# lmb-freiburg/demon

Measured on AMD Instinct MI355X. Metric: image-pairs/s full 3-iter DeMoN forward @256x192, higher is better.
Workload: dtype f32

## Files before the change

### demon_amd/_lib.py

```python
import ctypes
import os

HERE = os.path.dirname(os.path.abspath(__file__))
LIB_PATH = os.environ.get("DEMON_HIP_LIB", os.path.join(HERE, "libdemon_hip.so"))

c_float_p = ctypes.POINTER(ctypes.c_float)
c_int_p = ctypes.POINTER(ctypes.c_int)
c_int64_p = ctypes.POINTER(ctypes.c_int64)
c_uint8_p = ctypes.POINTER(ctypes.c_uint8)


class DemonOutputs(ctypes.Structure):
    _fields_ = [(name, c_float_p) for name in (
        "predict_flow5", "predict_conf5", "predict_flow2", "predict_conf2", "predict_depth2",
        "predict_normal2", "predict_rotation", "predict_translation", "predict_scale")]


class LanesEntry(ctypes.Structure):
    _fields_ = [("lanes", ctypes.c_int), ("placeholder_streams", ctypes.c_int), ("pairs_per_s", ctypes.c_float)]


class LanesResult(ctypes.Structure):
    _fields_ = [("lanes", ctypes.c_int), ("placeholder_streams", ctypes.c_int), ("pairs_per_s", ctypes.c_float),
                ("verified_pairs_per_s", ctypes.c_float), ("attempts", ctypes.c_int), ("ntable", ctypes.c_int), ("table", LanesEntry * 64)]
# ... 62 lines not shown
    "demon_upload_images_u8_async": (_I, [_P, _I, c_uint8_p, c_uint8_p]),
    "demon_op_prepare_inputs_u8": (_I, [_P, c_float_p, c_float_p, c_uint8_p, c_uint8_p, _I, _I, _I, _I, _I]),
    "demon_cloud_configure": (_I, [_P, ctypes.POINTER(ctypes.c_double), _I]),
    "demon_run_cloud": (_I, [_P, _I]),
    "demon_download_cloud": (_I, [_P, _I, c_float_p, c_float_p, c_uint8_p, c_int_p]),
    "demon_download_cloud_async": (_I, [_P, _I, c_float_p, c_float_p, c_uint8_p, c_int_p]),
    "demon_download_outputs_async": (_I, [_P, _I, ctypes.POINTER(DemonOutputs), c_float_p]),
    "demon_host_register": (_I, [ctypes.c_void_p, ctypes.c_int64]),
    "demon_host_unregister": (_I, [ctypes.c_void_p]),
    "demon_time_full": (_I, [_P, _I, _I, _I, c_float_p]),
    "demon_profile_full": (_I, [_P, _I, _I, _I, ctypes.POINTER(LaunchRecord), _I, c_int_p]),
    "demon_op_depth_to_flow": (_I, [_P, c_float_p, c_float_p, c_float_p, c_float_p, c_float_p, _I, _I, _I, _I, _I, _I]),
    "demon_op_flow_to_depth": (_I, [_P, c_float_p, c_float_p, c_float_p, c_float_p, c_float_p, _I, _I, _I, _I, _I, _I]),
    "demon_op_warp2d": (_I, [_P, c_float_p, c_float_p, c_float_p, _I, _I, _I, _I, _I, _I, _F]),
    "demon_op_leaky_relu": (_I, [_P, c_float_p, c_float_p, ctypes.c_int64, _F]),
    "demon_op_replace_nonfinite": (_I, [_P, c_float_p, c_float_p, ctypes.c_int64, _F]),
    "demon_op_scale_invariant_gradient": (_I, [_P, c_float_p, c_float_p, _I, _I, _I, c_int_p, c_float_p, _I, _F]),
    "demon_op_median3x3_downsample": (_I, [_P, c_float_p, c_float_p, _I, _I, _I]),
    "demon_op_depth_to_normals": (_I, [_P, c_float_p, c_float_p, c_float_p, _I, _I, _I, _I]),
    "demon_op_pointwise_l2_loss": (_I, [_P, c_float_p, c_float_p, c_float_p, _I, _I, _I, _I, ctypes.c_float]),
    "demon_op_conv2d": (_I, [_P, c_float_p, c_float_p, c_float_p, c_float_p] + [_I] * 12),
    "demon_op_deconv4x4s2": (_I, [_P, c_float_p, c_float_p, c_float_p, c_float_p] + [_I] * 6),
    "demon_op_dense": (_I, [_P, c_float_p, c_float_p, c_float_p, c_float_p] + [_I] * 4),
    "demon_op_point_cloud": (_I, [_P, c_float_p, c_float_p, c_uint8_p, c_int_p, c_float_p, c_float_p, c_uint8_p, c_float_p, c_float_p, c_float_p, c_float_p] + [_I] * 5),
    "demon_bench_layer": (_I, [_P] + [_I] * 13 + [c_float_p, ctypes.POINTER(ctypes.c_double)]),
    "demon_bench_ingest": (_I, [_P, _I, _I, _I, c_float_p, c_float_p]),
    "demon_bench_cloud": (_I, [_P, _I, _I, _I, c_float_p]),
    "demon_last_kernel": (_I, [ctypes.c_char_p, _I]),
    "demon_debug_check_guards": (_I, [_P, c_int_p]),
}

_lib = None


def load():
    global _lib
    if _lib is not None:
        return _lib
    if not os.path.exists(LIB_PATH):
        raise RuntimeError(
            "libdemon_hip.so not found at %s -- build it with `python -m demon_amd.build` "
            "(there is no CPU fallback for the DeMoN hot path)" % LIB_PATH)
    lib = ctypes.CDLL(LIB_PATH)
    for name, (restype, argtypes) in SIGNATURES.items():
        fn = getattr(lib, name)
        fn.restype = restype
# ... 4 lines not shown
```

### demon_amd/build.py

```python
import os
import subprocess
import sys
from concurrent.futures import ThreadPoolExecutor

HERE = os.path.dirname(os.path.abspath(__file__))
CSRC = os.path.join(HERE, "csrc")
OUT = os.path.join(HERE, "libdemon_hip.so")
SOURCES = ["demon_api.hip", "conv_mfma.hip", "conv_bf16.hip", "conv_patch.hip", "conv_small.hip", "conv_pair.hip", "conv_stream.hip", "conv_frag.hip", "conv_wino.hip", "conv_wino3.hip", "conv_wino4.hip", "dense_stream.hip", "conv_thin.hip", "conv_row.hip", "ops.hip", "ingest.hip", "pointcloud.hip"]
FLAGS = ["--offload-arch=gfx950", "-O3", "-std=c++17", "-fPIC", "-Wall", "-Wno-unused-function", "-Wno-unused-value", "-Wno-unused-result"]


def csrc_sha():
    import glob
    import hashlib
    h = hashlib.sha1()
    files = [os.path.join(CSRC, n) for n in sorted(SOURCES) if n != "demon_api.hip"] + [os.path.join(CSRC, "internal.h"), os.path.join(CSRC, "wino1d_tables.h")]
    files += sorted(glob.glob(os.path.join(HERE, "tuned", "*.json")))
    for path in files:
        with open(path, "rb") as f:
            h.update(f.read())
    return h.hexdigest()[:16]


def _hipcc():
    for cand in (os.environ.get("HIPCC"), "/opt/rocm/bin/hipcc", "hipcc"):
        if cand and (os.path.isabs(cand) and os.path.exists(cand) or not os.path.isabs(cand)):
            return cand
    return "hipcc"


def _needs_build(target, deps):
# ... 47 lines not shown
```

### demon_amd/csrc/conv_pair.hip

```cpp
#include "internal.h"

namespace demon {

typedef float floatx16 __attribute__((ext_vector_type(16)));
typedef float floatx4 __attribute__((ext_vector_type(4)));

template <int K, int S, int MB1, int MB2, int C1>
struct PairGeom {
    static constexpr int TH = 4, TW = 32;
    static constexpr int TWm = (TW - 1) * S + K;
    static constexpr int TWp = (TWm + 3) / 4 * 4;
    static constexpr int PH = (TH - 1) * S + K;
    static constexpr int N1 = TH * TWp;
    static constexpr int NB1 = (N1 + 31) / 32;
    static constexpr int NBW = (NB1 + 3) / 4;
    static constexpr int CKS1 = C1;
    static constexpr bool ONE1 = C1 == 6;
    static constexpr int CKS2 = K == 3 ? 8 : 2;
    static constexpr int KD1 = K * CKS1, KD2 = K * CKS2;
    static constexpr int PPS = PH * TWp;
    static constexpr int PELEMS = CKS1 * PPS;
    static constexpr int EPP = (PPS + 255) / 256;
    static constexpr int A1CH = KD1 * MB1 * 8, A1PER = (A1CH + 255) / 256;
    static constexpr int A2CH = KD2 * MB2 * 8, A2PER = (A2CH + 255) / 256;
// ... 246 lines not shown
                float v = acc2[i][r] + a.b2[co];
                v = v >= 0.0f ? v : 0.1f * v;
                ob[(long)co * plane] = v;
            }
        }
}

template <int K, int S, int MB1, int MB2, int C1>
static bool launch_pair_t(const PairArgs &a_in, hipStream_t s)
{
    using G = PairGeom<K, S, MB1, MB2, C1>;
    static PerDeviceOnce once;
    if (G::lds_bytes > 64 * 1024 &&
        !once.ensure([] { return hipFuncSetAttribute(reinterpret_cast<const void *>(&conv_pair_kernel<K, S, MB1, MB2, C1>), hipFuncAttributeMaxDynamicSharedMemorySize, (int)G::lds_bytes) == hipSuccess; }))
        return false;
    PairArgs a = a_in;
    a.steps1 = (a.Cin + C1 - 1) / C1;
    a.steps2 = (a.CM + G::CKS2 - 1) / G::CKS2;
    dim3 grid((unsigned)(a.N * a.tiles_y * a.tiles_x));
    hipLaunchKernelGGL((conv_pair_kernel<K, S, MB1, MB2, C1>), grid, dim3(256), G::lds_bytes, s, a);
    return true;
}

bool conv_pair_applies(int k, int stride, int cin, int cm, int co)
{
    static const int all = getenv("DEMON_FUSED_PAIRS_ALL") ? atoi(getenv("DEMON_FUSED_PAIRS_ALL")) : 0;
    const bool shape = (k == 9 && stride == 2) || (k == 7 && stride == 2) || (k == 3 && stride == 1);
    if (!shape || cm > 64 || co > 64 || cm % 8) return false;
    return all || (k == 9 && cin <= 16);
}

void conv_pair_tiles(int Ho, int Wo, int &tiles_y, int &tiles_x)
{
    tiles_y = (Ho + 3) / 4;
    tiles_x = (Wo + 31) / 32;
}

int conv_pair_cks(int k) { return k == 3 ? 8 : 2; }

bool launch_conv_pair(const PairArgs &a, int k, int stride, hipStream_t s)
{
    const int mb1 = (a.CM + 31) / 32, mb2 = (a.CO + 31) / 32;
    static const int one_step = getenv("DEMON_PAIR_ONE_STEP") ? atoi(getenv("DEMON_PAIR_ONE_STEP")) : 1;
    if (k == 9 && stride == 2 && a.Cin == 6 && mb1 == 1 && one_step) {
        if (mb2 == 1) return launch_pair_t<9, 2, 1, 1, 6>(a, s);
        return launch_pair_t<9, 2, 1, 2, 6>(a, s);
    }
#define PAIR_CASE(KK, SS, CC)                                                  \
    if (k == KK && stride == SS) {                                             \
        if (mb1 == 1 && mb2 == 1) return launch_pair_t<KK, SS, 1, 1, CC>(a, s); \
        if (mb1 == 1 && mb2 == 2) return launch_pair_t<KK, SS, 1, 2, CC>(a, s); \
        if (mb1 == 2 && mb2 == 1) return launch_pair_t<KK, SS, 2, 1, CC>(a, s); \
// ... 11 lines not shown
```

### demon_amd/csrc/demon_api.hip

```cpp
#include <hip/hip_runtime.h>
#include <dlfcn.h>
#include <rccl/rccl.h>
#include <stdio.h>
#include <stdlib.h>
#include <string.h>

#include <algorithm>
#include <cmath>
#include <array>
#include <chrono>
#include <functional>
#include <mutex>
#include <map>
#include <memory>
#include <string>
#include <vector>

#include "../../include/demon_hip.h"
#include "internal.h"

using namespace demon;

namespace {

// ... 1234 lines not shown
    if (const char *pk = getenv("DEMON_TUNE_PICK")) {
        const Cand &cd = cands[(size_t)atoi(pk) % cands.size()];
        best_t = Layer::Tuned{cd.kind, cd.tile, cd.ksplit};
    }
    L->tuned[n] = best_t;
    return DEMON_OK;
}

bool run_pair(const Layer *Ly, const Layer *Lx, int n, hipStream_t s)
{
    PairArgs a;
    a.in = Ly->in.ptr(); a.out = Lx->out.ptr();
    a.w1 = Ly->d_wp; a.b1 = Ly->d_bias; a.w2 = Lx->d_wp; a.b2 = Lx->d_bias;
    a.N = n; a.Cin = Ly->Cin; a.H = Ly->in.H; a.W = Ly->in.W; a.in_n_stride = Ly->in.n_stride();
    a.CM = Ly->Cout; a.CMk = Lx->Cin; a.CO = Lx->Cout; a.Mpad1 = Ly->Mpad; a.Mpad2 = Lx->Mpad;
    a.Hm = Ly->out.H; a.Ho = Lx->out.H; a.Wo = Lx->out.W; a.out_n_stride = Lx->out.n_stride();
    a.ph = Ly->ph; a.pw = Lx->pw;
    conv_pair_tiles(a.Ho, a.Wo, a.tiles_y, a.tiles_x);
    const int cks = conv_pair_cks(Ly->kh);
    a.steps1 = (a.Cin + cks - 1) / cks;
    a.steps2 = (a.CM + cks - 1) / cks;
    static const int xcd_order = getenv("DEMON_XCD_ORDER") ? atoi(getenv("DEMON_XCD_ORDER")) : 1;
    a.xcd = xcd_order;
    if (!launch_conv_pair(a, Ly->kh, Ly->sh, s)) return false;
    g_last_kernel = "conv_pair";
    return true;
}

bool chain_shape_ok(const Layer *Ly, const Layer *Lx, int kind, int v)
{
    if (!Ly->stream_ok() || !Lx->stream_ok() || Ly->kind != Layer::CONV || Lx->kind != Layer::CONV) return false;
    if (Ly->sh != 1 || Ly->sw != 1 || Lx->sh != 1 || Lx->sw != 1 || Lx->kh != 1 || Ly->Mpad != Lx->Mpad) return false;
    if (Ly->out.H != Lx->out.H || Ly->out.W != Lx->out.W || Ly->scale || Lx->scale) return false;
    if (kind == 6) return v >= 0 && v < FRAG_VARIANTS && frag_variant_kw(v) == 1 && frag_variant_bm(v) == Ly->Mpad && frag_variant_bn(v) % Ly->out.W == 0;
    if (kind == 7) return v >= 0 && v < STREAM_VARIANTS && stream_variant_kw(v) == 1 && stream_variant_bm(v) == Ly->Mpad && stream_variant_bn(v) % Ly->out.W == 0;
    return false;
}

bool chain_choice(const Layer *Ly, const Layer *Lx, int n, int &kind, int &v)
{
    if (const char *fp = getenv("DEMON_FORCE_PLAN")) {
        int ks = 0;
        if (sscanf(fp, "%d,%d,%d", &kind, &v, &ks) == 3) return (kind == 6 || kind == 7) && chain_shape_ok(Ly, Lx, kind, v);
    }
    auto it = nearest_tuned(Ly, n);
    if (it == Ly->tuned.end()) return false;
// ... 57 lines not shown
        st.kernel = "conv_mfma";
        const double pix = (kind == Layer::DECONV) ? 4.0 * in.H * in.W : (double)out.H * out.W;
        const double kreal = (kind == Layer::DECONV) ? 4.0 * in.C : (double)p->K;
        st.flops_per_sample = 2.0 * out.C * kreal * pix;
        st.bytes_per_sample = 4.0 * ((double)in.C * in.H * in.W + (double)out.C * out.H * out.W);
        st.bytes_fixed = 4.0 * ((double)p->K * p->ncls * out.C + out.C);
        float *ws = side ? c->d_ws_side : c->d_ws;
        st.fn = [p, ws](int n, hipStream_t s) { run_layer(p, n, s, ws); };
        st.image_only = tag;
        if (add_step) { stamp(st); steps->push_back(st); }
        return p;
    }
    Layer *conv(const std::string &name, View in, View out, int k, int stride, int act, const float *scale = nullptr)
    {
        return make(name, Layer::CONV, in, out, k, k, stride, stride, act, scale);
    }
    void conv2(const std::string &name, View in, View out, int k, int s, int cy = 0)
    {
        const int Hmid = (in.H + 2 * (k / 2) - k) / s + 1;
        if (!cy) cy = out.C;
        char key[64];
        snprintf(key, sizeof key, "tmp_y_%dx%dx%d", cy, Hmid, in.W);
        View mid = buffer(c, key, cy, Hmid, in.W);
        const bool fusable = conv_pair_applies(k, s, in.C, cy, out.C) && (long)out.H * out.W >= 2048;
        const bool chainable = !fusable && s == 1 && Layer::stream_shape_ok(Layer::CONV, in.C, k, 1) && Layer::stream_shape_ok(Layer::CONV, cy, 1, k) &&
                               (cy + 31) / 32 == (out.C + 31) / 32;
        if (!fusable && !chainable) {
            make(name + "y", Layer::CONV, in, mid, k, 1, s, 1, 1);
            make(name + "x", Layer::CONV, mid, out, 1, k, 1, s, 1);
            return;
        }
        const int jn = join_next, fk = fork_next;
        Layer *Ly = make(name + "y", Layer::CONV, in, mid, k, 1, s, 1, 1, nullptr, false);
        Layer *Lx = make(name + "x", Layer::CONV, mid, out, 1, k, 1, s, 1, nullptr, false);
        Step st;
        st.name = Ly->name + "+x";
        st.kernel = "conv_mfma";
        st.flops_per_sample = 2.0 * Ly->Cout * Ly->K * Ly->out.H * Ly->out.W + 2.0 * Lx->Cout * Lx->K * Lx->out.H * Lx->out.W;
        st.bytes_per_sample = 4.0 * ((double)in.C * in.H * in.W + (double)out.C * out.H * out.W);
        st.bytes_fixed = 4.0 * ((double)Ly->K * Ly->Cout + (double)Lx->K * Lx->Cout + Ly->Cout + Lx->Cout);
        float *ws = side ? c->d_ws_side : c->d_ws;
        std::function<bool(int)> applies;
        if (chainable) {
            c->chain_pairs.push_back({Ly, Lx});
            applies = [Ly, Lx](int n) { int kind, v; return !Ly->bf16_on() && !Lx->bf16_on() && chain_choice(Ly, Lx, n, kind, v); };
            st.bytes_per_sample += 8.0 * (double)cy * Hmid * in.W;
            st.fn = [Ly, Lx, ws](int n, hipStream_t s2) {
// ... 687 lines not shown
{
    if (!c || index < 0 || index >= (int)c->variables.size()) return DEMON_ERR_INVALID;
    const Variable &v = c->variables[index];
    if (name && name_cap > 0) { strncpy(name, v.name.c_str(), name_cap - 1); name[name_cap - 1] = 0; }
    for (int i = 0; i < 4; ++i) dims[i] = i < v.ndim ? v.dims[i] : 1;
    if (ndim) *ndim = v.ndim;
    return DEMON_OK;
}

int demon_set_weight(demon_ctx *c, const char *tf_name, const float *host, const int64_t *dims, int ndim)
{
    if (!c || !tf_name || !host) return fail(c, DEMON_ERR_INVALID, "null argument");
    auto it = c->var_index.find(tf_name);
    if (it == c->var_index.end()) return fail(c, DEMON_ERR_NOT_FOUND, std::string("unknown variable ") + tf_name);
    const Variable &v = c->variables[it->second];
    if (dims) {
        bool same = ndim == v.ndim;
        for (int i = 0; same && i < ndim; ++i) same = dims[i] == v.dims[i];
        if (!same) return fail(c, DEMON_ERR_INVALID, std::string("shape mismatch for variable ") + tf_name);
    }
    hipSetDevice(c->device);
    for (auto &g : c->graphs) hipGraphExecDestroy(g.second);
    c->graphs.clear();
    if (v.is_bias) {
        HIP_TRY(c, hipMemcpy(v.layer->d_bias, host, sizeof(float) * v.layer->Cout, hipMemcpyHostToDevice));
        v.layer->have_bias = true;
        return DEMON_OK;
    }
    return upload_kernel(c, v.layer, host);
}

int64_t demon_weights_blob_size(const demon_ctx *c)
{
    if (!c) return 0;
    int64_t total = 0;
    for (const Variable &v : c->variables) total += v.count;
    return total;
}

int demon_set_weights_blob(demon_ctx *c, const float *blob, int64_t nfloats)
{
    if (!c || !blob) return fail(c, DEMON_ERR_INVALID, "null argument");
    if (nfloats != demon_weights_blob_size(c)) return fail(c, DEMON_ERR_INVALID, "weight blob size mismatch");
    int64_t off = 0;
    for (const Variable &v : c->variables) {
        int r = demon_set_weight(c, v.name.c_str(), blob + off, v.dims, v.ndim);
// ... 106 lines not shown
    if (!nccl_comm || !nranks) return fail(nullptr, DEMON_ERR_INVALID, "null argument");
    if (!r.err.empty()) return rccl_fail(nullptr, "rccl", 0);
    int rc = r.CommCount((ncclComm_t)nccl_comm, nranks);
    return rc ? rccl_fail(nullptr, "ncclCommCount", rc) : DEMON_OK;
}
}
namespace {
uint64_t slab_layout_hash(const demon_ctx *c)
{
    uint64_t h = 1469598103934665603ull;
    auto mix = [&h](uint64_t v) { for (int i = 0; i < 8; ++i) { h ^= (v >> (8 * i)) & 0xff; h *= 1099511628211ull; } };
    mix((uint64_t)c->variant); mix((uint64_t)c->H); mix((uint64_t)c->W); mix((uint64_t)c->w_slab_floats);
    for (auto &L : c->layers) {
        for (char ch : L->name) mix((uint64_t)(unsigned char)ch);
        mix((uint64_t)L->ncls); mix((uint64_t)L->Krows); mix((uint64_t)L->Mpad);
        mix((uint64_t)(L->d_wp - c->w_slab)); mix((uint64_t)(L->d_bias - c->w_slab));
    }
    return h;
}
void slab_arrived(demon_ctx *c)
{
    for (auto &g : c->graphs) hipGraphExecDestroy(g.second);
    c->graphs.clear();
    for (auto &L : c->layers) { L->have_kernel = L->have_bias = true; L->wf_dirty = true; L->wb_dirty = true; L->w1_dirty = true; L->w3_dirty = true; L->w4_dirty = true; L->wd_dirty = true; }
}
}
extern "C" {

uint64_t demon_weights_slab_layout(const demon_ctx *c) { return c && c->w_slab ? slab_layout_hash(c) : 0; }

int demon_broadcast_weights(demon_ctx *c, void *nccl_comm, int root, int rank)
{
    if (!c || !nccl_comm) return fail(c, DEMON_ERR_INVALID, "null argument");
    if (!c->w_slab) return fail(c, DEMON_ERR_INVALID, "context has no networks (demon_create_ops)");
    if (!c->stream) return fail(c, DEMON_ERR_NOT_READY, kNoStream);
    RcclApi &r = rccl();
    if (!r.err.empty()) return rccl_fail(c, "rccl", 0);
    std::string missing;
    const bool root_ready = rank != root || weights_ready(c, &missing);
    hipSetDevice(c->device);
    HIP_TRY(c, hipStreamSynchronize(c->stream));
    TmpDev tmp;
    int *hdr = (int *)tmp.alloc(4);
    if (!hdr) return fail(c, DEMON_ERR_HIP, "temporary device allocation failed");
    const uint64_t mine = slab_layout_hash(c);
    int h_hdr[4] = {(int)(mine & 0xffffffffu), (int)(mine >> 32), root_ready ? 1 : 0, 0};
// ... 113 lines not shown
            run_layer(Ly, n, c->stream, c->d_ws);
            run_layer(Lx, n, c->stream, c->d_ws);
        }, failed);
    };
    const bool had = Ly->tuned.count(n) > 0;
    const Layer::Tuned before = had ? Ly->tuned[n] : Layer::Tuned{14, 0, 1};
    Ly->tuned[n] = Layer::Tuned{12, 0, 1};
    const float two = measure(false);
    const float one = measure(true);
    if (failed) return DEMON_ERR_HIP;
    if (one <= two) {
        Ly->tuned[n] = (had && before.kind != 12) ? before : Layer::Tuned{14, 0, 1};
    }
    return DEMON_OK;
}

int demon_autotune(demon_ctx *c, int n)
{
    if (!c || n < 1 || n > c->max_batch) return fail(c, DEMON_ERR_INVALID, "batch size out of range [1, max_batch]");
    if (!c->stream) return fail(c, DEMON_ERR_NOT_READY, kNoStream);
    hipSetDevice(c->device);
    for (auto &g : c->graphs) hipGraphExecDestroy(g.second);
    c->graphs.clear();
    struct KeepPrecision {
        demon_ctx *c;
        int saved;
        ~KeepPrecision() { c->opt_precision = saved; }
    } keep{c, c->opt_precision};
    c->opt_precision = 0;
    prepare_stream_weights(c);
    const char *only_env = getenv("DEMON_TUNE_ONLY");
    std::vector<std::string> only_list;
    for (std::string rest = only_env ? only_env : ""; !rest.empty();) {
        const size_t e = rest.find(',');
        if (e) only_list.push_back(rest.substr(0, e));
        rest = e == std::string::npos ? "" : rest.substr(e + 1);
    }
    struct OnlyFilter {
        const std::vector<std::string> &pats;
        bool any;
        bool skips(const std::string &name) const
        {
            if (!any) return false;
            for (const std::string &p : pats) if (name.find(p) != std::string::npos) return false;
            return true;
        }
// ... 16 lines not shown
    return DEMON_OK;
}

int demon_num_layers(const demon_ctx *c) { return c ? (int)c->layers.size() : 0; }

int demon_plan_get(const demon_ctx *c, int n, int layer_index, char *name, int name_cap, int *kind, int *tile, int *ksplit)
{
    if (!c || layer_index < 0 || layer_index >= (int)c->layers.size()) return DEMON_ERR_INVALID;
    const Layer *L = c->layers[layer_index].get();
    if (name && name_cap > 0) { strncpy(name, L->name.c_str(), name_cap - 1); name[name_cap - 1] = 0; }
    auto it = L->tuned.find(n);
    if (it == L->tuned.end()) return DEMON_ERR_NOT_FOUND;
    if (kind) *kind = it->second.kind;
    if (tile) *tile = it->second.tile;
    if (ksplit) *ksplit = it->second.ksplit;
    return DEMON_OK;
}

int demon_plan_clear(demon_ctx *c, int n)
{
    if (!c || n < 1 || n > c->max_batch) return fail(c, DEMON_ERR_INVALID, "batch size out of range [1, max_batch]");
    for (auto &g : c->graphs) hipGraphExecDestroy(g.second);
    c->graphs.clear();
    for (auto &L : c->layers) L->tuned.erase(n);
    return DEMON_OK;
}

int demon_plan_set(demon_ctx *c, int n, const char *layer_name, int kind, int tile, int ksplit)
{
    if (!c || !layer_name || n < 1 || n > c->max_batch) return fail(c, DEMON_ERR_INVALID, "bad argument");
    if (kind < 0 || kind > 16 || kind == 2 || kind == 9 || tile < 0 ||
        tile >= (kind == 16 ? (int)WINO4_VARIANTS : kind == 15 ? (int)WINO3_VARIANTS : kind >= 12 ? 1 : kind == 11 ? (int)DENSE_VARIANTS : kind == 10 ? (int)WINO1D_VARIANTS : kind == 8 ? (int)WINO_VARIANTS : (kind == 1 ? (int)PTILE_COUNT : ((kind == 4 || kind == 7) ? (int)STREAM_VARIANTS : ((kind == 5 || kind == 6) ? (int)FRAG_VARIANTS : (int)TILE_COUNT)))) || ksplit < 0)
        return fail(c, DEMON_ERR_INVALID, "bad plan entry");
    if (kind != 1 && ksplit >= 1000)
        return fail(c, DEMON_ERR_INVALID, "ksplit >= 1000 is only meaningful for the patch-staged kernel (pixel-tile shape)");
    for (auto &L : c->layers)
        if (L->name == layer_name) {
            if (kind == 0 && L->Mpad % conv_tile_bm(tile)) return fail(c, DEMON_ERR_INVALID, "tile does not divide Cout");
            if (kind == 3 && !small_applies(L.get())) return fail(c, DEMON_ERR_INVALID, "the small-Cout kernel does not apply to this layer");
            if (kind == 8 && !wino_applies(L.get())) return fail(c, DEMON_ERR_INVALID, "the minimal-filtering kernel applies to transposed convs only");
            if (kind == 10 && !wino1d_applies(L.get())) return fail(c, DEMON_ERR_INVALID, "no 1-D minimal-filtering form for this layer");
            if (kind == 16 && !wino4_applies(L.get())) return fail(c, DEMON_ERR_INVALID, "conv_wino4.hip applies to k x 1 / 1 x k convs with 3 taps stride 1 or 5 taps stride 2 and >= 16 input channels only");
            if (kind == 15 && !wino3_applies(L.get())) return fail(c, DEMON_ERR_INVALID, "conv_wino3.hip applies to 3 x 3 convs with >= 16 input channels, stride 1 (rows of even length) or stride 2 (rows of a multiple of 8 pixels, >= 64)");
            if (kind == 13 && !row_applies(L.get())) return fail(c, DEMON_ERR_INVALID, "conv_row.hip applies to 1 x 7 / 1 x 9 stride-2 convs with at most 32 channels on both sides only");
            if (kind == 12 && !thin_applies(L.get())) return fail(c, DEMON_ERR_INVALID, "conv_thin.hip applies to the 9 x 1 stride-2 first layer (Cin <= 6, Cout <= 32) only");
            if (kind == 11 && !dense_stream_applies(L.get())) return fail(c, DEMON_ERR_INVALID, "the weight-streaming kernel applies to dense layers only");
            if (kind == 4 && (!L->stream_ok() || L->Mpad % stream_variant_bm(tile))) return fail(c, DEMON_ERR_INVALID, "the streaming kernel does not apply to this layer");
            if (kind == 5 && (!L->stream_ok() || L->Mpad % frag_variant_bm(tile))) return fail(c, DEMON_ERR_INVALID, "the fragment-tiled kernel does not apply to this layer");
            if (kind == 6 || kind == 7) {
                bool ok = false;
                for (auto &pr : c->chain_pairs) ok = ok || (pr.first == L.get() && chain_shape_ok(pr.first, pr.second, kind, tile));
                if (!ok) return fail(c, DEMON_ERR_INVALID, "this layer cannot run chained with a 1 x k partner on that variant");
            }
            for (auto &g : c->graphs) hipGraphExecDestroy(g.second);
            c->graphs.clear();
            L->tuned[n] = Layer::Tuned{kind, tile, (kind == 0 || kind == 4 || kind == 5) && ksplit < 1 ? 1 : ksplit};
            return DEMON_OK;
        }
    return fail(c, DEMON_ERR_NOT_FOUND, std::string("unknown layer ") + layer_name);
}

int demon_upload_inputs(demon_ctx *c, int n, const float *image_pair, const float *image2_2)
{
    int r = check_batch(c, n);
    if (r) return r;
    hipSetDevice(c->device);
    if ((r = h2d(c, c->image_pair, image_pair, n))) return r;
    if ((r = h2d(c, c->image2_2, image2_2, n))) return r;
    HIP_TRY(c, hipStreamSynchronize(c->stream));
    return DEMON_OK;
}

int demon_upload_inputs_async(demon_ctx *c, int n, const float *image_pair, const float *image2_2)
{
    int r = check_batch(c, n);
    if (r) return r;
    hipSetDevice(c->device);
    if ((r = h2d(c, c->image_pair, image_pair, n))) return r;
// ... 1003 lines not shown
}

int demon_op_conv2d(demon_ctx *c, float *out, const float *in, const float *w_hwio, const float *bias, int n, int cin, int h,
                    int w, int cout, int kh, int kw, int sh, int sw, int ph, int pw, int lrelu)
{
    const bool same = ph == -1 && pw == -1;
    if (c && !same && (ph != kh / 2 || pw != kw / 2))
        return fail(c, DEMON_ERR_INVALID, "padding must be k/2 (helpers.py:78-79) or -1,-1 for TF 'same' (v2/helpers.py:24-35)");
    return run_single_layer(c, Layer::CONV, out, in, w_hwio, bias, n, cin, h, w, cout, kh, kw, sh, sw, lrelu, same);
}

int demon_op_deconv4x4s2(demon_ctx *c, float *out, const float *in, const float *w_hwoi, const float *bias, int n, int cin,
                         int h, int w, int cout, int lrelu)
{
    return run_single_layer(c, Layer::DECONV, out, in, w_hwoi, bias, n, cin, h, w, cout, 4, 4, 2, 2, lrelu);
}

int demon_op_dense(demon_ctx *c, float *out, const float *in, const float *w_io, const float *bias, int n, int cin, int cout,
                   int lrelu)
{
    return run_single_layer(c, Layer::DENSE, out, in, w_io, bias, n, cin, 1, 1, cout, 1, 1, 1, 1, lrelu);
}

}
```

### demon_amd/csrc/internal.h

```cpp
#pragma once
#include <hip/hip_runtime.h>
#include <stdint.h>

#include <atomic>
#include <string>
#include <vector>

namespace demon {

struct PerDeviceOnce {
    std::atomic<unsigned long long> done{0};
    template <class F>
    bool ensure(F &&configure)
    {
        int dev = 0;
        if (hipGetDevice(&dev) != hipSuccess || dev < 0 || dev > 63) return configure();
        if (done.load(std::memory_order_acquire) >> dev & 1ull) return true;
        if (!configure()) return false;
        done.fetch_or(1ull << dev, std::memory_order_release);
        return true;
    }
};

struct View {
// ... 179 lines not shown
int patch_tile_mtiles(int tile, int Cout, int Mpad);
int patch_tile_bm(int tile);
int patch_tile_bn(int tile);
int patch_tile_threads(int tile);
size_t patch_lds_bytes(int tile, int ntaps, int G, int PS);
void launch_conv_patch(const PatchArgs &a, int tile, int ntaps, int nclasses, hipStream_t stream);

struct PairArgs {
    const float *in;
    float *out;
    const float *w1, *b1;
    const float *w2, *b2;
    int N, Cin, H, W;
    long in_n_stride;
    int CM, CMk, CO, Mpad1, Mpad2;
    int Hm;
    int Ho, Wo;
    long out_n_stride;
    int ph, pw;
    int tiles_y, tiles_x;
    int steps1, steps2;
    int xcd;
};
bool conv_pair_applies(int k, int stride, int cin, int cm, int co);
void conv_pair_tiles(int Ho, int Wo, int &tiles_y, int &tiles_x);
int conv_pair_cks(int k);
bool launch_conv_pair(const PairArgs &a, int k, int stride, hipStream_t s);

struct WinoArgs {
    const float *in;
    float *out;
    const float *wp;
    const float *bias;
    float *ws;
    int N, Cin, H, W;
    long in_n_stride;
    int Cout, Mpad;
    long cls_w_stride;
    int Ho, Wo;
    long out_n_stride, out_plane;
    int act, ksplit, nsteps_total;
    int G, TY, TX, tiles_y, tiles_x;
    int PH, PW, PS;
    int xcd;
    unsigned m_plane, m_pw, m_tytx, m_tx, m_tilesx, m_tilesy;
};
constexpr int WINO_VARIANTS = 7;
int wino_variant_kh(int v);
int wino_variant_tn(int v);
int wino_variant_mb(int v);
// ... 219 lines not shown
```

### demon_amd/engine.py

```python
import ctypes

import numpy as np

from . import _lib
from ._lib import DemonOutputs, LaunchRecord, c_float_p, c_int_p, c_int64_p, c_uint8_p


class DemonError(ValueError):
    """Raised for every non-zero demon_status (the reference raises ValueError / InvalidArgumentError)."""


def _fp(a):
    return a.ctypes.data_as(c_float_p)


def _f32(a, shape=None, name="array"):
    a = np.ascontiguousarray(a, dtype=np.float32)
    if shape is not None and tuple(a.shape) != tuple(shape):
        raise DemonError("%s has shape %s, expected %s" % (name, tuple(a.shape), tuple(shape)))
    return a


def _u8p(a):
    return a.ctypes.data_as(c_uint8_p)
# ... 501 lines not shown
        self._check(self.lib.demon_op_conv2d(self.h, _fp(out), _fp(x), _fp(w_hwio), _fp(bias), n, cin, h, w, cout, kh, kw,
                                             sh, sw, ph, pw, int(lrelu)))
        return out

    def deconv4x4s2(self, x, w_hwoi, bias, lrelu=False):
        x, w_hwoi, bias = _f32(x), _f32(w_hwoi), _f32(bias)
        n, cin, h, w = x.shape
        if w_hwoi.shape[:2] != (4, 4) or w_hwoi.shape[3] != cin:
            raise DemonError("deconv4x4s2: weight must be [4,4,Cout,Cin]")
        cout = w_hwoi.shape[2]
        out = np.empty((n, cout, 2 * h, 2 * w), np.float32)
        self._check(self.lib.demon_op_deconv4x4s2(self.h, _fp(out), _fp(x), _fp(w_hwoi), _fp(bias), n, cin, h, w, cout,
                                                  int(lrelu)))
        return out

    def dense(self, x, w_io, bias, lrelu=False):
        x, w_io, bias = _f32(x), _f32(w_io), _f32(bias)
        n, cin = x.shape
        cout = w_io.shape[1]
        out = np.empty((n, cout), np.float32)
        self._check(self.lib.demon_op_dense(self.h, _fp(out), _fp(x), _fp(w_io), _fp(bias), n, cin, cout, int(lrelu)))
        return out

    def last_kernel(self):
        buf = ctypes.create_string_buffer(64)
        self.lib.demon_last_kernel(buf, 64)
        return buf.value.decode()

    def bench_ingest(self, n, warmup=5, iters=20):
        k, c = np.zeros(iters, np.float32), np.zeros(iters, np.float32)
        self._check(self.lib.demon_bench_ingest(self.h, int(n), int(warmup), int(iters), _fp(k), _fp(c)))
        return k.tolist(), c.tolist()

    def bench_cloud(self, n, warmup=5, iters=20):
        k = np.zeros(iters, np.float32)
        self._check(self.lib.demon_bench_cloud(self.h, int(n), int(warmup), int(iters), _fp(k)))
        return k.tolist()

    def bench_layer(self, kind, n, cin, h, w, cout, kh=1, kw=1, sh=1, sw=1, tile=-1, ksplit=0, iters=20):
        k = {"conv": 0, "deconv": 1, "dense": 2}[kind]
        ms = ctypes.c_float()
        fl = ctypes.c_double()
        self._check(self.lib.demon_bench_layer(self.h, k, n, cin, h, w, cout, kh, kw, sh, sw, tile, ksplit, iters,
                                               ctypes.byref(ms), ctypes.byref(fl)))
        return float(ms.value), fl.value / (ms.value * 1e-3) / 1e12
```

### demon_amd/kernel_names.py

```python
import functools
import os
import re

CSRC = os.path.join(os.path.dirname(os.path.abspath(__file__)), "csrc")


@functools.lru_cache(None)
def frag_variants():
    src = open(os.path.join(CSRC, "conv_frag.hip")).read()
    table = {}
    for m in re.finditer(r"case (\d+): launch_frag_instance<([\d, ]+)>", src):
        table[int(m.group(1))] = tuple(int(x) for x in m.group(2).split(","))
    m = re.search(r"default: launch_frag_instance<([\d, ]+)>", src)
    if m:
        table[max(table) + 1] = tuple(int(x) for x in m.group(1).split(","))
    return table


def kernel_tag(name):
    m = re.search(r"conv_mfma_kernel<(\d+), (\d+)", name)
    if m:
        return "conv_mfma<%sx%s>" % m.groups()
    m = re.search(r"conv_bf16_kernel<(\d+), (\d+)", name)
    if m:
# ... 50 lines not shown
            shapes4 = {(2, 2, 2, 2): 8, (4, 1, 2, 2): 9, (2, 2, 3, 1): 10, (4, 1, 3, 1): 11, (1, 4, 2, 1): 12, (1, 4, 3, 1): 13, (2, 1, 2, 2): 14, (4, 2, 3, 1): 15}
            return "wino3rows<f4t3x3,v%d>" % shapes4.get(shape, -1)
        shapes3 = {(2, 2, 4, 1): 0, (2, 4, 4, 1): 1, (4, 1, 4, 1): 2, (4, 2, 4, 1): 3, (1, 4, 4, 1): 4, (1, 4, 2, 2): 5, (2, 2, 2, 2): 6, (4, 1, 2, 2): 7}
        return "wino3rows<t3x3,v%d>" % shapes3.get(shape, -1)
    m = re.search(r"wino4_kernel<(\d+), (\d+), (\d+), (\d+), (\d+), (\d+), (true|false), (true|false), (true|false)", name)
    if m:
        kind, axis, wm, wn, tn, kg = map(int, m.groups()[:6])
        shapes4 = {(4, 1, 4, 1): 0, (4, 1, 2, 2): 1, (2, 2, 4, 1): 2, (2, 2, 2, 2): 3, (4, 2, 2, 2): 4, (4, 2, 4, 1): 5, (4, 1, 1, 4): 6, (2, 2, 1, 4): 7, (2, 2, 2, 1): 8,
                   (4, 2, 3, 2): 9, (2, 2, 3, 2): 10, (4, 1, 3, 2): 11, (2, 2, 3, 1): 12, (4, 2, 3, 1): 13}
        return "wino4<t%d,v%d%s>" % (3 if kind == 0 else 5, shapes4.get((wm, wn, tn, kg), -1), ",walk" if m.group(9) == "true" else "")
    m = re.search(r"conv_row_kernel<(\d+), ", name)
    if m:
        return "conv_row<32x128,t%d>" % (3 + 2 * int(m.group(1)))
    m = re.search(r"conv_thin_kernel<(\d+)", name)
    if m:
        return "conv_thin<32x512,t%s>" % m.group(1)
    m = re.search(r"dense_stream_kernel<(true|false)", name)
    if m:
        return "dense_stream<128x32,v%d>" % (1 if m.group(1) == "true" else 0)
    m = re.search(r"deconv4_kernel<(\d+), (\d+), (\d+)", name)
    if m:
        bm, wm, wn = map(int, m.groups())
        return "deconv4<%dx%d>" % (bm, wn * 32)
    m = re.search(r"demon::(\w+?)_kernel", name)
    return m.group(1) if m else name.split("(")[0]


def rocprof_kernel_name(tag):
    base = tag.split("+")[0]
    fam, _, rest = base.partition("<")
    dims = rest.rstrip(">").split(",")[0].split("x") if rest else []
    if fam == "conv_mfma" and len(dims) == 2:
        return "demon::conv_mfma_kernel<%s, %s, ...>" % tuple(dims)
    if fam == "conv_bf16" and len(dims) == 2:
        return "demon::conv_bf16_kernel<%s, %s, ...>" % tuple(dims)
    if fam == "conv_patch" and len(dims) == 2:
        return "demon::conv_patch_kernel<%s, ...> (%sx%s tile, %s taps)" % (dims[0], dims[0], dims[1], rest.rstrip(">").split(",t")[-1])
    if fam == "wino_deconv" and len(dims) == 2:
        kh2 = ",kh2" in rest
        return "demon::wino_deconv_kernel<%d, ..., %d, %d> (%s channels x %s tiles per workgroup%s)" % (
            int(dims[1]) // 16, int(dims[0]) // 16, 2 if kh2 else 1, dims[0], dims[1], ", reduction split in two inside the workgroup" if kh2 else "")
    if fam == "wino4":
        return "demon::wino4_kernel<...> (%s)" % rest.rstrip(">")
    if fam == "wino3rows":
        return "demon::wino3_rows_kernel<...> (%s)" % rest.rstrip(">")
    if fam == "wino1d":
# ... 22 lines not shown
```

### include/demon_hip.h

```cpp
#ifndef DEMON_HIP_H
#define DEMON_HIP_H

#include <stdint.h>

#ifdef __cplusplus
extern "C" {
#endif

typedef struct demon_ctx demon_ctx;

enum demon_status {
    DEMON_OK = 0,
    DEMON_ERR_INVALID = -1,
    DEMON_ERR_HIP = -2,
    DEMON_ERR_NOT_READY = -3,
    DEMON_ERR_NOT_FOUND = -4
};

typedef struct demon_outputs {
    float *predict_flow5;
    float *predict_conf5;
    float *predict_flow2;
    float *predict_conf2;
    float *predict_depth2;
// ... 113 lines not shown
                               int src_h, int src_w, int H, int W);
int demon_op_point_cloud(demon_ctx *ctx, float *points, float *normals, uint8_t *colors, int *counts, const float *depth,
                         const float *normals_in, const uint8_t *colors_u8_in, const float *image_in, const float *K, const float *R,
                         const float *t, int n, int h, int w, int inverse_depth, int color_rounding);
int demon_op_pointwise_l2_loss(demon_ctx *ctx, float *loss, const float *inp, const float *gt, int n, int c, int h, int w,
                               float epsilon);

#define DEMON_COMM_ID_BYTES 128
int demon_comm_get_unique_id(char *id );
int demon_comm_init_rank(void **nccl_comm, int nranks, const char *id , int rank, int device);
int demon_comm_destroy(void *nccl_comm);
int demon_broadcast_weights(demon_ctx *ctx, void *nccl_comm, int root, int rank);
int64_t demon_weights_slab_bytes(const demon_ctx *ctx);
uint64_t demon_weights_slab_layout(const demon_ctx *ctx);
int demon_comm_count(void *nccl_comm, int *nranks);
int demon_copy_weights_from(demon_ctx *dst, const demon_ctx *src);

int demon_op_conv2d(demon_ctx *ctx, float *out, const float *in, const float *w_hwio, const float *bias, int n,
                    int cin, int h, int w, int cout, int kh, int kw, int sh, int sw, int ph, int pw, int lrelu);
int demon_op_deconv4x4s2(demon_ctx *ctx, float *out, const float *in, const float *w_hwoi, const float *bias,
                         int n, int cin, int h, int w, int cout, int lrelu);
int demon_op_dense(demon_ctx *ctx, float *out, const float *in, const float *w_io, const float *bias, int n,
                   int cin, int cout, int lrelu);

int demon_bench_layer(demon_ctx *ctx, int kind, int n, int cin, int h, int w, int cout, int kh, int kw, int sh,
                      int sw, int tile, int ksplit, int iters, float *avg_ms, double *flops);

int demon_bench_ingest(demon_ctx *ctx, int n, int warmup, int iters, float *kernel_ms, float *copy_ms);

int demon_bench_cloud(demon_ctx *ctx, int n, int warmup, int iters, float *kernel_ms);

int demon_debug_check_guards(demon_ctx *ctx, int *violations);

int demon_last_kernel(char *tag, int tag_cap);

#ifdef __cplusplus
}
#endif
#endif
```

Before: 4651.

## Add row-band fused kernel for small 3x1/1x3 separable conv pairs

Adds a dedicated fused kernel for 3-tap stride-1 separable conv pairs with at most 9 input channels, 32 intermediate channels and widths up to 64. It processes a 4-row band per block, keeping the intermediate activation in LDS and the weights in registers, and runs both convolutions with MFMA. The fusion eligibility rule is widened so these pairs avoid writing and re-reading the intermediate tensor through global memory. It also adds a standalone conv_pair op for testing and clears group graphs on weight or plan changes. The extra LDS use and the two-blocks-per-CU launch bound may limit occupancy.

```diff
diff --git a/demon_amd/_lib.py b/demon_amd/_lib.py
--- a/demon_amd/_lib.py
+++ b/demon_amd/_lib.py
@@ -108,6 +108,7 @@
     "demon_op_conv2d": (_I, [_P, c_float_p, c_float_p, c_float_p, c_float_p] + [_I] * 12),
     "demon_op_deconv4x4s2": (_I, [_P, c_float_p, c_float_p, c_float_p, c_float_p] + [_I] * 6),
     "demon_op_dense": (_I, [_P, c_float_p, c_float_p, c_float_p, c_float_p] + [_I] * 4),
+    "demon_op_conv_pair": (_I, [_P] + [c_float_p] * 6 + [_I] * 10),
     "demon_op_point_cloud": (_I, [_P, c_float_p, c_float_p, c_uint8_p, c_int_p, c_float_p, c_float_p, c_uint8_p, c_float_p, c_float_p, c_float_p, c_float_p] + [_I] * 5),
     "demon_bench_layer": (_I, [_P] + [_I] * 13 + [c_float_p, ctypes.POINTER(ctypes.c_double)]),
     "demon_bench_ingest": (_I, [_P, _I, _I, _I, c_float_p, c_float_p]),
diff --git a/demon_amd/build.py b/demon_amd/build.py
--- a/demon_amd/build.py
+++ b/demon_amd/build.py
@@ -6,7 +6,7 @@
 HERE = os.path.dirname(os.path.abspath(__file__))
 CSRC = os.path.join(HERE, "csrc")
 OUT = os.path.join(HERE, "libdemon_hip.so")
-SOURCES = ["demon_api.hip", "conv_mfma.hip", "conv_bf16.hip", "conv_patch.hip", "conv_small.hip", "conv_pair.hip", "conv_stream.hip", "conv_frag.hip", "conv_wino.hip", "conv_wino3.hip", "conv_wino4.hip", "dense_stream.hip", "conv_thin.hip", "conv_row.hip", "ops.hip", "ingest.hip", "pointcloud.hip"]
+SOURCES = ["demon_api.hip", "conv_mfma.hip", "conv_bf16.hip", "conv_patch.hip", "conv_small.hip", "conv_pair.hip", "conv_pair_rows.hip", "conv_stream.hip", "conv_frag.hip", "conv_wino.hip", "conv_wino3.hip", "conv_wino4.hip", "dense_stream.hip", "conv_thin.hip", "conv_row.hip", "ops.hip", "ingest.hip", "pointcloud.hip"]
 FLAGS = ["--offload-arch=gfx950", "-O3", "-std=c++17", "-fPIC", "-Wall", "-Wno-unused-function", "-Wno-unused-value", "-Wno-unused-result"]
 
 
diff --git a/demon_amd/csrc/conv_pair.hip b/demon_amd/csrc/conv_pair.hip
--- a/demon_amd/csrc/conv_pair.hip
+++ b/demon_amd/csrc/conv_pair.hip
@@ -292,12 +292,12 @@
     return true;
 }
 
-bool conv_pair_applies(int k, int stride, int cin, int cm, int co)
+bool conv_pair_applies(int k, int stride, int cin, int cm, int co, int w)
 {
     static const int all = getenv("DEMON_FUSED_PAIRS_ALL") ? atoi(getenv("DEMON_FUSED_PAIRS_ALL")) : 0;
     const bool shape = (k == 9 && stride == 2) || (k == 7 && stride == 2) || (k == 3 && stride == 1);
     if (!shape || cm > 64 || co > 64 || cm % 8) return false;
-    return all || (k == 9 && cin <= 16);
+    return all || (k == 9 && cin <= 16) || (k == 3 && cin <= 9 && cm == 32 && co == 32 && w <= 64 && w % 4 == 0);
 }
 
 void conv_pair_tiles(int Ho, int Wo, int &tiles_y, int &tiles_x)
diff --git a/demon_amd/csrc/conv_pair_rows.hip b/demon_amd/csrc/conv_pair_rows.hip
--- /dev/null
+++ b/demon_amd/csrc/conv_pair_rows.hip
@@ -0,0 +1,160 @@
+#include "internal.h"
+
+namespace demon {
+
+typedef float floatx4 __attribute__((ext_vector_type(4)));
+
+constexpr int P3_ROWS = 4, P3_W = 64, P3_NT = 256;
+constexpr int P3_CIN = 9;
+constexpr int P3_PH = P3_ROWS + 2;
+constexpr int P3_MP = 80;
+constexpr int P3_PS = P3_PH * P3_MP + 16;
+constexpr int P3_PATCH = P3_CIN * P3_PS;
+constexpr int P3_SLAB = 32 * P3_MP;
+constexpr size_t P3_LDS = sizeof(float) * (size_t)(P3_PATCH + P3_ROWS * P3_SLAB);
+
+__global__ __launch_bounds__(P3_NT, 2) void conv_pair_rows_kernel(PairArgs a)
+{
+    extern __shared__ __attribute__((aligned(16))) float smem[];
+    float *patch = smem;
+    const int tid = threadIdx.x, lane = tid & 63, l15 = lane & 15, lk = lane >> 4;
+    const int wave = __builtin_amdgcn_readfirstlane(tid >> 6);
+    float *midw = smem + P3_PATCH + wave * P3_SLAB;
+    unsigned bx, by;
+    xcd_tile(a.xcd, blockIdx.x, 0, gridDim.x, 1, bx, by);
+    const int n = bx / a.tiles_y, band = bx - n * a.tiles_y;
+    const int y0 = band * P3_ROWS;
+    const float *__restrict__ in0 = a.in + (long)n * a.in_n_stride;
+
+    const int nrows = a.Cin * P3_PH;
+    constexpr int MAXP = (P3_CIN * P3_PH * (P3_W / 4) + P3_NT - 1) / P3_NT;
+    floatx4 pv[MAXP];
+#pragma unroll
+    for (int i = 0; i < MAXP; ++i) {
+        const int e = tid + i * P3_NT, row = e >> 4, xq = e & 15;
+        const int ci = row / P3_PH, pr = row - ci * P3_PH;
+        const int gy = y0 - 1 + pr;
+        const bool ok = row < nrows && (unsigned)gy < (unsigned)a.H && 4 * xq < a.W;
+        pv[i] = floatx4{0.0f, 0.0f, 0.0f, 0.0f};
+        if (ok) pv[i] = *reinterpret_cast<const floatx4 *>(in0 + ((long)ci * a.H + gy) * a.W + 4 * xq);
+    }
+
+    float w1r[7][2], w2r[24][2];
+    int koff[7];
+    bool kv[7];
+    const int K1 = 3 * a.Cin;
+#pragma unroll
+    for (int s = 0; s < 7; ++s) {
+        const int k = 4 * s + lk;
+        kv[s] = k < K1;
+        const int ci = kv[s] ? k / 3 : 0, tap = kv[s] ? k - ci * 3 : 0;
+        koff[s] = ci * P3_PS + tap * P3_MP;
+#pragma unroll
+        for (int cb = 0; cb < 2; ++cb) w1r[s][cb] = kv[s] ? a.w1[(long)(tap * a.Cin + ci) * a.Mpad1 + cb * 16 + l15] : 0.0f;
+    }
+#pragma unroll
+    for (int s = 0; s < 24; ++s)
+#pragma unroll
+        for (int cb = 0; cb < 2; ++cb) w2r[s][cb] = a.w2[(long)(4 * s + lk) * a.Mpad2 + cb * 16 + l15];
+
+#pragma unroll
+    for (int i = 0; i < MAXP; ++i) {
+        const int e = tid + i * P3_NT, row = e >> 4, xq = e & 15;
+        const int ci = row / P3_PH, pr = row - ci * P3_PH;
+        if (row < nrows) *reinterpret_cast<floatx4 *>(patch + ci * P3_PS + pr * P3_MP + 4 * xq) = pv[i];
+    }
+    midw[(lane & 31) * P3_MP + (lane < 32 ? 0 : a.W + 1)] = 0.0f;
+    __syncthreads();
+
+    const int ntx = (a.W + 15) >> 4;
+
+    floatx4 acc[4][2];
+#pragma unroll
+    for (int t = 0; t < 4; ++t)
+#pragma unroll
+        for (int cb = 0; cb < 2; ++cb) acc[t][cb] = floatx4{0.0f, 0.0f, 0.0f, 0.0f};
+#pragma unroll
+    for (int s = 0; s < 7; ++s) {
+        const float *p = patch + wave * P3_MP + l15 + koff[s];
+        float b[4];
+#pragma unroll
+        for (int t = 0; t < 4; ++t) b[t] = kv[s] ? p[t * 16] : 0.0f;
+#pragma unroll
+        for (int t = 0; t < 4; ++t)
+            if (t < ntx) {
+#pragma unroll
+                for (int cb = 0; cb < 2; ++cb) acc[t][cb] = __builtin_amdgcn_mfma_f32_16x16x4f32(w1r[s][cb], b[t], acc[t][cb], 0, 0, 0);
+            }
+    }
+#pragma unroll
+    for (int t = 0; t < 4; ++t)
+        if (t < ntx) {
+            const int x = 16 * t + l15;
+#pragma unroll
+            for (int cb = 0; cb < 2; ++cb)
+#pragma unroll
+                for (int r = 0; r < 4; ++r) {
+                    const int cm = cb * 16 + 4 * lk + r;
+                    float v = acc[t][cb][r] + a.b1[cm];
+                    v = v >= 0.0f ? v : 0.1f * v;
+                    midw[cm * P3_MP + 1 + x] = x < a.W ? v : 0.0f;
+                }
+        }
+    __syncthreads();
+
+#pragma unroll
+    for (int t = 0; t < 4; ++t)
+#pragma unroll
+        for (int cb = 0; cb < 2; ++cb) acc[t][cb] = floatx4{0.0f, 0.0f, 0.0f, 0.0f};
+#pragma unroll
+    for (int s = 0; s < 24; ++s) {
+        const float *p = midw + (4 * (s & 7) + lk) * P3_MP + (s >> 3) + l15;
+        float b[4];
+#pragma unroll
+        for (int t = 0; t < 4; ++t) b[t] = t < ntx ? p[t * 16] : 0.0f;
+#pragma unroll
+        for (int t = 0; t < 4; ++t)
+            if (t < ntx) {
+#pragma unroll
+                for (int cb = 0; cb < 2; ++cb) acc[t][cb] = __builtin_amdgcn_mfma_f32_16x16x4f32(w2r[s][cb], b[t], acc[t][cb], 0, 0, 0);
+            }
+    }
+
+    const int y = y0 + wave;
+    if (y >= a.Ho) return;
+    const long plane = (long)a.Ho * a.Wo;
+    float *__restrict__ ob = a.out + (long)n * a.out_n_stride + (long)y * a.Wo;
+#pragma unroll
+    for (int t = 0; t < 4; ++t) {
+        const int x = 16 * t + l15;
+        if (t < ntx && x < a.Wo) {
+#pragma unroll
+            for (int cb = 0; cb < 2; ++cb)
+#pragma unroll
+                for (int r = 0; r < 4; ++r) {
+                    const int co = cb * 16 + 4 * lk + r;
+                    if (co < a.CO) {
+                        float v = acc[t][cb][r] + a.b2[co];
+                        v = v >= 0.0f ? v : 0.1f * v;
+                        ob[co * plane + x] = v;
+                    }
+                }
+        }
+    }
+}
+
+bool conv_pair_rows_shape_ok(const PairArgs &a, int k, int stride)
+{
+    return k == 3 && stride == 1 && a.ph == 1 && a.pw == 1 && a.Cin >= 1 && a.Cin <= P3_CIN && a.CM == 32 && a.CMk == 32 && a.Mpad1 == 32 &&
+           a.CO >= 1 && a.CO <= 32 && a.Mpad2 == 32 && a.W >= 4 && a.W <= P3_W && (a.W & 3) == 0 && a.Hm == a.H && a.Ho == a.H && a.Wo == a.W &&
+           (a.in_n_stride & 3) == 0 && (reinterpret_cast<uintptr_t>(a.in) & 15) == 0;
+}
+
+void launch_conv_pair_rows(PairArgs a, hipStream_t s)
+{
+    a.tiles_y = (a.Ho + P3_ROWS - 1) / P3_ROWS;
+    a.tiles_x = 1;
+    hipLaunchKernelGGL(conv_pair_rows_kernel, dim3((unsigned)(a.N * a.tiles_y)), dim3(P3_NT), P3_LDS, s, a);
+}
+
+}
diff --git a/demon_amd/csrc/demon_api.hip b/demon_amd/csrc/demon_api.hip
--- a/demon_amd/csrc/demon_api.hip
+++ b/demon_amd/csrc/demon_api.hip
@@ -1280,6 +1280,12 @@
     a.steps2 = (a.CM + cks - 1) / cks;
     static const int xcd_order = getenv("DEMON_XCD_ORDER") ? atoi(getenv("DEMON_XCD_ORDER")) : 1;
     a.xcd = xcd_order;
+    static const int pair_rows = getenv("DEMON_PAIR_ROWS") ? atoi(getenv("DEMON_PAIR_ROWS")) : 1;
+    if (pair_rows && conv_pair_rows_shape_ok(a, Ly->kh, Ly->sh)) {
+        launch_conv_pair_rows(a, s);
+        g_last_kernel = "conv_pair";
+        return true;
+    }
     if (!launch_conv_pair(a, Ly->kh, Ly->sh, s)) return false;
     g_last_kernel = "conv_pair";
     return true;
@@ -1383,7 +1389,7 @@
         char key[64];
         snprintf(key, sizeof key, "tmp_y_%dx%dx%d", cy, Hmid, in.W);
         View mid = buffer(c, key, cy, Hmid, in.W);
-        const bool fusable = conv_pair_applies(k, s, in.C, cy, out.C) && (long)out.H * out.W >= 2048;
+        const bool fusable = conv_pair_applies(k, s, in.C, cy, out.C, in.W) && (long)out.H * out.W >= 2048;
         const bool chainable = !fusable && s == 1 && Layer::stream_shape_ok(Layer::CONV, in.C, k, 1) && Layer::stream_shape_ok(Layer::CONV, cy, 1, k) &&
                                (cy + 31) / 32 == (out.C + 31) / 32;
         if (!fusable && !chainable) {
@@ -2117,6 +2123,7 @@
     hipSetDevice(c->device);
     for (auto &g : c->graphs) hipGraphExecDestroy(g.second);
     c->graphs.clear();
+    drop_group_graphs(c);
     if (v.is_bias) {
         HIP_TRY(c, hipMemcpy(v.layer->d_bias, host, sizeof(float) * v.layer->Cout, hipMemcpyHostToDevice));
         v.layer->have_bias = true;
@@ -2269,6 +2276,7 @@
 {
     for (auto &g : c->graphs) hipGraphExecDestroy(g.second);
     c->graphs.clear();
+    drop_group_graphs(c);
     for (auto &L : c->layers) { L->have_kernel = L->have_bias = true; L->wf_dirty = true; L->wb_dirty = true; L->w1_dirty = true; L->w3_dirty = true; L->w4_dirty = true; L->wd_dirty = true; }
 }
 }
@@ -2428,6 +2436,7 @@
     hipSetDevice(c->device);
     for (auto &g : c->graphs) hipGraphExecDestroy(g.second);
     c->graphs.clear();
+    drop_group_graphs(c);
     struct KeepPrecision {
         demon_ctx *c;
         int saved;
@@ -2490,6 +2499,7 @@
     if (!c || n < 1 || n > c->max_batch) return fail(c, DEMON_ERR_INVALID, "batch size out of range [1, max_batch]");
     for (auto &g : c->graphs) hipGraphExecDestroy(g.second);
     c->graphs.clear();
+    drop_group_graphs(c);
     for (auto &L : c->layers) L->tuned.erase(n);
     return DEMON_OK;
 }
@@ -2522,6 +2532,7 @@
             }
             for (auto &g : c->graphs) hipGraphExecDestroy(g.second);
             c->graphs.clear();
+            drop_group_graphs(c);
             L->tuned[n] = Layer::Tuned{kind, tile, (kind == 0 || kind == 4 || kind == 5) && ksplit < 1 ? 1 : ksplit};
             return DEMON_OK;
         }
@@ -3571,4 +3582,52 @@
     return run_single_layer(c, Layer::DENSE, out, in, w_io, bias, n, cin, 1, 1, cout, 1, 1, 1, 1, lrelu);
 }
 
-}
+int demon_op_conv_pair(demon_ctx *c, float *out, const float *in, const float *w1_hwio, const float *b1, const float *w2_hwio,
+                       const float *b2, int n, int cin, int h, int w, int cmid, int cout, int k, int stride, int out_channels, int out_c0)
+{
+    if (!c) return DEMON_ERR_INVALID;
+    hipSetDevice(c->device);
+    if (!out || !in || !w1_hwio || !b1 || !w2_hwio || !b2 || n < 1 || cin < 1 || h < 1 || w < 1 || out_c0 < 0 || cout < 1 || out_c0 + cout > out_channels)
+        return fail(c, DEMON_ERR_INVALID, "bad argument");
+    const bool shape = (k == 9 && stride == 2) || (k == 7 && stride == 2) || (k == 3 && stride == 1);
+    if (!shape || cmid < 8 || cmid > 64 || cmid % 8 || cout > 64)
+        return fail(c, DEMON_ERR_INVALID, "the fused pair exists for 9 / 7 taps stride 2 and 3 taps stride 1, up to 64 channels (intermediate: a multiple of 8)");
+    if (!c->stream) return fail(c, DEMON_ERR_NOT_READY, kNoStream);
+    demon_ctx scratch;
+    scratch.device = c->device;
+    scratch.max_batch = n;
+    scratch.guard_bytes = guard_bytes_from_env();
+    const int hm = (h + 2 * (k / 2) - k) / stride + 1, wo = (w + 2 * (k / 2) - k) / stride + 1;
+    Layer Ly, Lx;
+    Ly.kind = Lx.kind = Layer::CONV;
+    Ly.Cin = cin; Ly.Cout = cmid; Ly.kh = k; Ly.kw = 1; Ly.sh = stride; Ly.sw = 1; Ly.ph = k / 2; Ly.pw = 0; Ly.act = 1;
+    Lx.Cin = cmid; Lx.Cout = cout; Lx.kh = 1; Lx.kw = k; Lx.sh = 1; Lx.sw = stride; Lx.ph = 0; Lx.pw = k / 2; Lx.act = 1;
+    Ly.in = buffer(&scratch, "in", cin, h, w);
+    Ly.out = Lx.in = buffer(&scratch, "mid", cmid, hm, w);
+    const View whole = buffer(&scratch, "out", out_channels, hm, wo);
+    Lx.out = whole.slice(out_c0, cout);
+    const size_t nout = (size_t)n * out_channels * hm * wo;
+    int rc = DEMON_OK;
+    if (!Ly.in.base || !Ly.out.base || !whole.base || !plan_layer(&scratch, &Ly) || !plan_layer(&scratch, &Lx))
+        rc = fail(c, DEMON_ERR_HIP, scratch.err.empty() ? std::string("temporary device allocation failed") : scratch.err);
+    if (!rc && (upload_kernel(&scratch, &Ly, w1_hwio) || upload_kernel(&scratch, &Lx, w2_hwio))) rc = fail(c, DEMON_ERR_HIP, scratch.err);
+    if (!rc && (hipMemcpy(Ly.d_bias, b1, sizeof(float) * cmid, hipMemcpyHostToDevice) != hipSuccess ||
+                hipMemcpy(Lx.d_bias, b2, sizeof(float) * cout, hipMemcpyHostToDevice) != hipSuccess ||
+                hipMemcpy(Ly.in.base, in, sizeof(float) * (size_t)n * cin * h * w, hipMemcpyHostToDevice) != hipSuccess ||
+                hipMemcpy(whole.base, out, sizeof(float) * nout, hipMemcpyHostToDevice) != hipSuccess))
+        rc = fail(c, DEMON_ERR_HIP, "upload failed");
+    if (!rc) {
+        if (!run_pair(&Ly, &Lx, n, c->stream)) rc = fail(c, DEMON_ERR_INVALID, "no fused kernel for this pair");
+        else if (hipGetLastError() != hipSuccess || hipStreamSynchronize(c->stream) != hipSuccess ||
+                 hipMemcpy(out, whole.base, sizeof(float) * nout, hipMemcpyDeviceToHost) != hipSuccess)
+            rc = fail(c, DEMON_ERR_HIP, "pair execution failed");
+    }
+    if (!rc && scratch.guard_bytes) {
+        std::string where;
+        if (check_guards(&scratch, &where)) rc = fail(c, DEMON_ERR_HIP, std::string("poison harness: a kernel wrote outside its tensors (") + (g_last_kernel ? g_last_kernel : "?") + "): " + where);
+    }
+    for (void *p : scratch.allocations) hipFree(p);
+    return rc;
+}
+
+}
diff --git a/demon_amd/csrc/internal.h b/demon_amd/csrc/internal.h
--- a/demon_amd/csrc/internal.h
+++ b/demon_amd/csrc/internal.h
@@ -225,10 +225,12 @@
     int steps1, steps2;
     int xcd;
 };
-bool conv_pair_applies(int k, int stride, int cin, int cm, int co);
+bool conv_pair_applies(int k, int stride, int cin, int cm, int co, int w);
 void conv_pair_tiles(int Ho, int Wo, int &tiles_y, int &tiles_x);
 int conv_pair_cks(int k);
 bool launch_conv_pair(const PairArgs &a, int k, int stride, hipStream_t s);
+bool conv_pair_rows_shape_ok(const PairArgs &a, int k, int stride);
+void launch_conv_pair_rows(PairArgs a, hipStream_t s);
 
 struct WinoArgs {
     const float *in;
diff --git a/demon_amd/engine.py b/demon_amd/engine.py
--- a/demon_amd/engine.py
+++ b/demon_amd/engine.py
@@ -547,6 +547,22 @@
         self._check(self.lib.demon_op_dense(self.h, _fp(out), _fp(x), _fp(w_io), _fp(bias), n, cin, cout, int(lrelu)))
         return out
 
+    def conv_pair(self, x, w1_hwio, b1, w2_hwio, b2, stride=1, out=None, out_c0=0):
+        x, w1_hwio, b1, w2_hwio, b2 = _f32(x), _f32(w1_hwio), _f32(b1), _f32(w2_hwio), _f32(b2)
+        n, cin, h, w = x.shape
+        k, one, ci, cmid = w1_hwio.shape
+        if one != 1 or ci != cin or w2_hwio.shape[:3] != (1, k, cmid) or b1.shape != (cmid,) or b2.shape != (w2_hwio.shape[3],):
+            raise DemonError("conv_pair: weight / bias shape mismatch")
+        cout = w2_hwio.shape[3]
+        ho, wo = (h + 2 * (k // 2) - k) // stride + 1, (w + 2 * (k // 2) - k) // stride + 1
+        if out is None:
+            out = np.zeros((n, cout, ho, wo), np.float32)
+        if out.dtype != np.float32 or not out.flags.c_contiguous or out.shape[0] != n or out.shape[2:] != (ho, wo):
+            raise DemonError("conv_pair: out must be a C-contiguous float32 [n, C, %d, %d] array" % (ho, wo))
+        self._check(self.lib.demon_op_conv_pair(self.h, _fp(out), _fp(x), _fp(w1_hwio), _fp(b1), _fp(w2_hwio), _fp(b2), n, cin, h, w,
+                                                cmid, cout, k, int(stride), out.shape[1], int(out_c0)))
+        return out
+
     def last_kernel(self):
         buf = ctypes.create_string_buffer(64)
         self.lib.demon_last_kernel(buf, 64)
diff --git a/demon_amd/kernel_names.py b/demon_amd/kernel_names.py
--- a/demon_amd/kernel_names.py
+++ b/demon_amd/kernel_names.py
@@ -96,6 +96,8 @@
     if m:
         bm, wm, wn = map(int, m.groups())
         return "deconv4<%dx%d>" % (bm, wn * 32)
+    if "conv_pair_rows_kernel" in name:
+        return "conv_pair"
     m = re.search(r"demon::(\w+?)_kernel", name)
     return m.group(1) if m else name.split("(")[0]
 
diff --git a/include/demon_hip.h b/include/demon_hip.h
--- a/include/demon_hip.h
+++ b/include/demon_hip.h
@@ -159,6 +159,9 @@
                          int n, int cin, int h, int w, int cout, int lrelu);
 int demon_op_dense(demon_ctx *ctx, float *out, const float *in, const float *w_io, const float *bias, int n,
                    int cin, int cout, int lrelu);
+int demon_op_conv_pair(demon_ctx *ctx, float *out, const float *in, const float *w1_hwio, const float *b1, const float *w2_hwio,
+                       const float *b2, int n, int cin, int h, int w, int cmid, int cout, int k, int stride, int out_channels,
+                       int out_c0);
 
 int demon_bench_layer(demon_ctx *ctx, int kind, int n, int cin, int h, int w, int cout, int kh, int kw, int sh,
                       int sw, int tile, int ksplit, int iters, float *avg_ms, double *flops);
```

Result: no change. 4656 (median of 4 runs) (+0.1%).
